# MartinMikkelsen/TensorTrainNumerics.jl

Hardware: AMD Instinct MI355X
Metric: TT cores/sec for QTT Laplacian apply+round, d=30 rank-64 (higher is better)
Workload: dtype f64

## Files before the change

tensortrainnumerics.jl_amd/csrc/ttn_eig_kernels.h:

```cpp
#pragma once
#include "ttn_dense_kernels.h"

#define EIG_N 128
template <int J>
__device__ __forceinline__ void fmac_bcast(double& a, double w, double s_) {
    asm volatile("v_fmac_f64_dpp %0, %1, %2 row_newbcast:%3 row_mask:0xf bank_mask:0xf" : "+v"(a) : "v"(w), "v"(s_), "n"(J));
}
#define EIG_BCAST16(M) M(0) M(1) M(2) M(3) M(4) M(5) M(6) M(7) M(8) M(9) M(10) M(11) M(12) M(13) M(14) M(15)
#define EIG_TAIL TTN_LDS_IMG

__device__ __forceinline__ void lds_barrier() { asm volatile("s_waitcnt lgkmcnt(0)\n\ts_barrier" ::: "memory"); }
__device__ __forceinline__ double wave64_sum_mfma(double v) {
    v = grp_sum(v);
    v += dpp_mov_f64<0x124>(v);
    v += dpp_mov_f64<0x128>(v);
    return v;
}
__device__ __forceinline__ double readlane_f64(double v, int idx) {
    union { double d; int i[2]; } u, r;
    u.d = v;
    r.i[0] = __builtin_amdgcn_readlane(u.i[0], idx);
    r.i[1] = __builtin_amdgcn_readlane(u.i[1], idx);
    return r.d;
}

template <int N>
__device__ __noinline__ void wg_tridiag(const double* Gg, int ldg, double* Vst, double* lds) {
    Gg = unip(Gg); Vst = unip(Vst); lds = unip(lds); ldg = uni32(ldg);
    constexpr bool TWO = (N == 128);
    constexpr int CW = (N * N / 16 > TTN_WG) ? 32 : 16;
    constexpr int NH = CW / 16;
    constexpr int NC = N / CW;
    static_assert(N * NC <= TTN_WG, "one thread per (row, column chunk)");
    lds_f64* L = (lds_f64*)lds;
    lds_f64 *vbuf0 = L, *vbuf1 = L + 128, *wL = L + 256, *xnext = L + 384, *part = L + 512;
    lds_f64 *dg = L + EIG_TAIL, *e = dg + 128, *beta = dg + 384;
    const int tid = threadIdx.x, lane = tid & 63, wave = tid >> 6;
    const int i = tid & (N - 1), c = tid / N;
    const bool actv = tid < N * NC;
    double a[CW];
#pragma unroll
    for (int j = 0; j < CW; ++j) a[j] = actv ? Gg[i + (long long)ldg * (CW * c + j)] : 0.0;
    lds_f64* xt = L + 1664;
    if (actv && i == 0) {
#pragma unroll
        for (int j = 0; j < CW; ++j) wL[CW * c + j] = a[j];
    }
    if (actv && i == 1) {
#pragma unroll
        for (int j = 0; j < CW; ++j) xnext[CW * c + j] = a[j];
    }
    __syncthreads();
    double rx0 = 0.0, rx1 = 0.0, ralpha = 0.0, rden = 0.0, rdg = 0.0;
    if (wave == 0) {
        rx0 = (lane > 0) ? wL[lane] : 0.0; rx1 = TWO ? wL[lane + 64] : 0.0;
        const double xk1 = wL[1];
        rdg = wL[0];
        xt[lane] = rx0; xt[lane + 64] = rx1;
        const double s2 = wave64_sum_mfma(fma(rx0, rx0, rx1 * rx1));
        ralpha = (s2 > 0.0) ? -copysign(s2 * fast_rsqrt2(s2), xk1) : 0.0;
        rden = s2 - ralpha * xk1;
    }
    for (int k = 0; k < N - 2; ++k) {
        lds_f64* vL = (k & 1) ? vbuf1 : vbuf0;
        lds_barrier();
        const bool live = actv && (CW * (c + 1) > k + 1) && ((TWO ? 64 * (wave & 1) : 0) + 63 > k);
        double v0 = 0.0, v1 = 0.0, w0 = 0.0, w1 = 0.0, bta = 0.0;
        if (wave == 0) {
            __builtin_amdgcn_s_setprio(TTN_TRIDIAG_PRIO);
            if (rden > 0.0) { bta = fast_rcp(rden); bta = fma(fma(-rden, bta, 1.0), bta, bta); }
            v0 = rx0 - ((lane == k + 1) ? ralpha : 0.0); v1 = rx1 - ((lane + 64 == k + 1) ? ralpha : 0.0);
            vL[lane] = v0; vL[lane + 64] = v1;
            typedef __attribute__((address_space(1))) double gdouble;
            gdouble* vg = (gdouble*)(unsigned long long)(Vst + k * 128);
            vg[lane] = v0; vg[lane + 64] = v1;
            if (lane == 0) { dg[k] = rdg; e[k] = ralpha; beta[k] = bta; }
        }
        if (live) {
            double xreg[NH];
#pragma unroll
            for (int h = 0; h < NH; ++h) xreg[h] = xt[CW * c + 16 * h + (lane & 15)];
            double pp = 0.0;
            asm volatile("s_nop 1");
#define EIG_MV(j) fmac_bcast<j>(pp, xreg[0], a[j]);
            EIG_BCAST16(EIG_MV)
#undef EIG_MV
            if constexpr (NH == 2) {
#define EIG_MV(j) fmac_bcast<j>(pp, xreg[1], a[16 + j]);
                EIG_BCAST16(EIG_MV)
#undef EIG_MV
            }
            part[c * 128 + i] = pp;
        } else if (actv) part[c * 128 + i] = 0.0;
        lds_barrier();
        lds_f64* xn_r = (k & 1) ? xnext + 1152 : xnext;
        lds_f64* xn_w = (k & 1) ? xnext : xnext + 1152;
        if (wave == 0) {
            double p0 = 0.0, p1 = 0.0;
#pragma unroll
            for (int cc = 0; cc < NC; ++cc) { p0 += part[cc * 128 + lane]; if (TWO) p1 += part[cc * 128 + lane + 64]; }
            p0 = bta * fma(-ralpha, xn_r[lane], p0); p1 = TWO ? bta * fma(-ralpha, xn_r[lane + 64], p1) : 0.0;
            const double Kc = 0.5 * bta * wave64_sum_mfma(fma(p0, v0, p1 * v1));
            w0 = fma(-Kc, v0, p0); w1 = fma(-Kc, v1, p1);
            wL[lane] = w0; if (TWO) wL[lane + 64] = w1;
        }
        lds_barrier();
        if (wave == 0 && k + 1 < N - 2) {
            const double wk1 = wL[k + 1], vk1 = vL[k + 1];
            const double c0 = fma(-v0, wk1, fma(-w0, vk1, xn_r[lane]));
            const double c1 = TWO ? fma(-v1, wk1, fma(-w1, vk1, xn_r[lane + 64])) : 0.0;
            const int kk = k + 1;
            rdg = (kk < 64) ? readlane_f64(c0, kk) : readlane_f64(c1, kk - 64);
            const double xk1 = (kk + 1 < 64) ? readlane_f64(c0, kk + 1) : readlane_f64(c1, kk + 1 - 64);
            rx0 = (lane > kk) ? c0 : 0.0; rx1 = (TWO && lane + 64 > kk) ? c1 : 0.0;
            xt[lane] = rx0; xt[lane + 64] = rx1;
            const double s2 = wave64_sum_mfma(fma(rx0, rx0, rx1 * rx1));
            ralpha = (s2 > 0.0) ? -copysign(s2 * fast_rsqrt2(s2), xk1) : 0.0;
            rden = s2 - ralpha * xk1;
        }
        if (wave == 0) __builtin_amdgcn_s_setprio(TTN_EIG_PRIO);
        if (live) {
            double vreg[NH], wreg[NH];
#pragma unroll
            for (int h = 0; h < NH; ++h) { vreg[h] = vL[CW * c + 16 * h + (lane & 15)]; wreg[h] = wL[CW * c + 16 * h + (lane & 15)]; }
            const double nvi = -vL[i], nwi = -wL[i];
            asm volatile("s_nop 1");
#define EIG_UP(j) fmac_bcast<j>(a[j], wreg[0], nvi); fmac_bcast<j>(a[j], vreg[0], nwi);
            EIG_BCAST16(EIG_UP)
#undef EIG_UP
            if constexpr (NH == 2) {
#define EIG_UP(j) fmac_bcast<j>(a[16 + j], wreg[1], nvi); fmac_bcast<j>(a[16 + j], vreg[1], nwi);
                EIG_BCAST16(EIG_UP)
#undef EIG_UP
            }
            if (i == k + 2) {
#pragma unroll
                for (int j = 0; j < CW; ++j) xn_w[CW * c + j] = a[j];
            }
        }
    }
    __syncthreads();
    if (actv && i == N - 2 && c == NC - 1) { dg[N - 2] = a[CW - 2]; e[N - 2] = a[CW - 1]; }
    if (actv && i == N - 1 && c == NC - 1) { dg[N - 1] = a[CW - 1]; }
    __syncthreads();
}

template <int N>
__device__ __forceinline__ int sturm_count(const double (&dreg)[N / 16], const double (&ereg)[N / 16], double x, bool& zero) {
    double pc = 1.0, pp = 0.0;
    const double nx = -x, one = 1.0;
    int cnt = 0;
    bool z = false;
    unsigned int prev = 0;
#pragma unroll
    for (int g = 0; g < N / 16; ++g) {
        unsigned int bits = 0;
#define EIG_ST(j) {                                                                                               \
            double dmx = nx;                                                                                      \
            fmac_bcast<j>(dmx, dreg[g], one);                                         \
            double pn = dmx * pc;                                                                                 \
            fmac_bcast<j>(pn, ereg[g], pp);                        \
            z |= (pn == 0.0);                                                                                     \
            bits = __builtin_amdgcn_alignbit(bits, (unsigned int)(__double_as_longlong(pn) >> 32), 31);           \
            pp = pc; pc = pn; }
        EIG_BCAST16(EIG_ST)
#undef EIG_ST
        const unsigned int seq = (prev << 16) | (bits & 0xffffu);
        cnt += __popc((seq ^ (seq >> 1)) & 0xffffu);
        prev = bits & 1u;
        const double ap = fabs(pc);
        if (ap < 0x1p-400 || ap > 0x1p400) {
            const double sc = (ap < 1.0) ? 0x1p500 : 0x1p-500;
            pc *= sc; pp *= sc;
        }
    }
    zero = z;
    return cnt;
}
__device__ __noinline__ int sturm_count_guarded(const lds_f64* de, double x, int n) {
    double pc = 1.0, pp = 0.0;
    int cnt = 0;
    for (int i = 0; i < n; ++i) {
        double pn = fma(de[2 * i] - x, pc, de[2 * i + 1] * pp);
        if (pn == 0.0) pn = copysign(DBL_MIN, -pc);
        cnt += (int)(((unsigned long long)(__double_as_longlong(pn) ^ __double_as_longlong(pc))) >> 63);
        pp = pc; pc = pn;
        const double ap = fabs(pc);
        if (ap < 0x1p-400 || ap > 0x1p400) { const double sc = (ap < 1.0) ? 0x1p500 : 0x1p-500; pc *= sc; pp *= sc; }
    }
    return cnt;
}

template <int N, int TL>
__device__ void wg_bisect(int nev, double* lds) {
    lds_f64* L = (lds_f64*)lds;
    lds_f64 *dg = L + EIG_TAIL, *e = dg + 128, *lam = dg + 256;
    lds_f64* e2 = L;
    const int tid = threadIdx.x;
    lds_f64* de = L + 256;
    for (int t = tid; t < N; t += TTN_WG) { e2[t] = (t < N - 1) ? e[t] * e[t] : 0.0; de[2 * t] = dg[t]; de[2 * t + 1] = (t > 0) ? -(e[t - 1] * e[t - 1]) : 0.0; }
    __syncthreads();
    if (tid < 64) {
        double glo_ = 1e300, ghi_ = -1e300, emax_ = 0.0;
        for (int t = tid; t < N; t += 64) {
            const double rad = ((t > 0) ? fabs(e[t - 1]) : 0.0) + ((t < N - 1) ? fabs(e[t]) : 0.0);
            glo_ = fmin(glo_, dg[t] - rad); ghi_ = fmax(ghi_, dg[t] + rad);
            emax_ = fmax(emax_, e2[t]);
        }
        glo_ = -wave_max(-glo_); ghi_ = wave_max(ghi_); emax_ = wave_max(emax_);
        if (tid == 0) { e2[128] = glo_; e2[129] = ghi_; e2[130] = emax_; }
    }
    __syncthreads();
    double glo = e2[128], ghi = e2[129];
    const double emax = e2[130];
    const double span = fmax(fabs(glo), fabs(ghi));
    glo -= 2.0 * DBL_EPSILON * span * N; ghi += 2.0 * DBL_EPSILON * span * N;
    const double pivmin = DBL_MIN * fmax(1.0, emax);
    double dreg[N / 16], ereg[N / 16];
#pragma unroll
    for (int g = 0; g < N / 16; ++g) { dreg[g] = de[2 * (16 * g + (tid & 15))]; ereg[g] = de[2 * (16 * g + (tid & 15)) + 1]; }
    asm volatile("s_nop 1");
    for (int g0 = 0; g0 < nev; g0 += TTN_WG / TL) {
        const int gi = g0 + tid / TL, sub = tid % TL;
        const bool act = gi < nev;
        const int jasc = N - 1 - (act ? gi : 0);
        double lo = glo, hi = ghi;
        for (int round = 0; round < 64; ++round) {
            const double wdt = hi - lo;
            const bool done = !(wdt > 2.0 * DBL_EPSILON * fmax(fabs(lo), fabs(hi)) + 2.0 * pivmin);
            if (__syncthreads_and(done || !act)) break;
            const double x = lo + wdt * ((double)(sub + 1) / (double)(TL + 1));
            const bool wave_act = g0 + (tid & ~63) / TL < nev;
            bool zero = false;
            int cnt = wave_act ? sturm_count<N>(dreg, ereg, x, zero) : 0;
            if (zero) cnt = sturm_count_guarded(de, x, N);
            int nf = (cnt <= jasc) ? 1 : 0;
#pragma unroll
            for (int m = 1; m < TL; m <<= 1) nf += __shfl_xor(nf, m);
            if (!done) {
                const double nlo = (nf > 0) ? lo + wdt * ((double)nf / (double)(TL + 1)) : lo;
                const double nhi = (nf < TL) ? lo + wdt * ((double)(nf + 1) / (double)(TL + 1)) : hi;
                lo = nlo; hi = nhi;
            }
        }
        if (act && sub == 0) lam[gi] = 0.5 * (lo + hi);
    }
    __syncthreads();
}

template <int N>
struct EigDm {
    static constexpr bool IN_LDS = 2 * N * 64 <= TTN_LDS_IMG;
    typedef __attribute__((address_space(1))) double gdouble;
    lds_f64* l;
    gdouble* g;
    __device__ __forceinline__ double ld(int idx) const { if constexpr (IN_LDS) return l[idx]; else return g[idx]; }
    __device__ __forceinline__ void st(int idx, double v) const { if constexpr (IN_LDS) l[idx] = v; else g[idx] = v; }
};
template <int N>
__device__ void wg_twisted(int r, double* lds, int* tw , lds_f64* zn , double* Dmg) {
    lds_f64* L = (lds_f64*)lds;
    lds_f64 *dg = L + EIG_TAIL, *e = dg + 128, *lam = dg + 256;
    lds_f64* Dp = L;
    EigDm<N> Dm;
    Dm.l = L + N * 64; Dm.g = (typename EigDm<N>::gdouble*)(unsigned long long)Dmg;
    const int tid = threadIdx.x, lane = tid & 63, wave = tid >> 6;
    double emax = 0.0;
    for (int t = 0; t < N - 1; ++t) emax = fmax(emax, e[t] * e[t]);
    const double pivmin = DBL_MIN * fmax(1.0, emax);
    __syncthreads();
    const bool act = lane < r;
    const double lm = lam[act ? lane : 0];
    if (wave == 0) {
        double q = 1.0;
        for (int i0 = 0; i0 < N; i0 += 8) {
            double dd[8], ee[8];
#pragma unroll
            for (int t = 0; t < 8; ++t) { dd[t] = dg[i0 + t]; ee[t] = (i0 + t > 0) ? e[i0 + t - 1] : 0.0; }
#pragma unroll
            for (int t = 0; t < 8; ++t) {
                q = fma(-(ee[t] * ee[t]), fast_rcp(q), dd[t] - lm);
                if (fabs(q) < pivmin) q = -pivmin;
                Dp[(i0 + t) * 64 + lane] = q;
            }
        }
    } else if (wave == 1) {
        double q = 1.0;
        for (int i0 = N - 8; i0 >= 0; i0 -= 8) {
            double dd[8], ee[8];
#pragma unroll
            for (int t = 0; t < 8; ++t) { dd[t] = dg[i0 + t]; ee[t] = (i0 + t < N - 1) ? e[i0 + t] : 0.0; }
#pragma unroll
            for (int t = 7; t >= 0; --t) {
                q = fma(-(ee[t] * ee[t]), fast_rcp(q), dd[t] - lm);
                if (fabs(q) < pivmin) q = -pivmin;
                Dm.st((i0 + t) * 64 + lane, q);
            }
        }
    }
    __syncthreads();
    if (wave < 2) {
        double gbest = 1e300;
        int kb = 0;
        for (int i0 = 0; i0 < N; i0 += 8) {
            double dm[8];
#pragma unroll
            for (int t = 0; t < 8; ++t) dm[t] = Dm.ld((i0 + t) * 64 + lane);
#pragma unroll
            for (int t = 0; t < 8; ++t) {
                const double g = fabs(Dp[(i0 + t) * 64 + lane] + dm[t] - (dg[i0 + t] - lm));
                if (g < gbest) { gbest = g; kb = i0 + t; }
            }
        }
        double z = 1.0, nrm = 0.0;
        if (wave == 0) {
            for (int i = kb - 1; i >= 0; --i) {
                z = -(e[i] * fast_rcp(Dp[i * 64 + lane])) * z;
                Dp[i * 64 + lane] = z;
                nrm = fma(z, z, nrm);
            }
            if (act) { tw[lane] = kb; zn[lane] = nrm; }
        } else {
            if constexpr (EigDm<N>::IN_LDS) {
                for (int i = kb; i < N - 1; ++i) {
                    z = -(e[i] * fast_rcp(Dm.ld((i + 1) * 64 + lane))) * z;
                    Dm.st((i + 1) * 64 + lane, z);
                    nrm = fma(z, z, nrm);
                }
            } else {
                for (int i0 = 0; i0 < N - 1; i0 += 8) {
                    double dm[8];
#pragma unroll
                    for (int t = 0; t < 8; ++t) dm[t] = (i0 + t + 1 < N) ? Dm.ld((i0 + t + 1) * 64 + lane) : 1.0;
#pragma unroll
                    for (int t = 0; t < 8; ++t) {
                        const int i = i0 + t;
                        if (i >= kb && i < N - 1) {
                            z = -(e[i] * fast_rcp(dm[t])) * z;
                            Dm.st((i + 1) * 64 + lane, z);
                            nrm = fma(z, z, nrm);
                        }
                    }
                }
            }
            if (act) zn[64 + lane] = nrm;
        }
    }
    __syncthreads();
    if (tid < 64 && tid < r) zn[tid] = 1.0 / sqrt(1.0 + zn[tid] + zn[64 + tid]);
    __syncthreads();
}

template <int N>
__device__ __noinline__ int wg_eig_n(const double* Gg, int ldg, double* Vst, int r, int nev, double* sig, double* lds, int* iwork ,
                                     double* dwork ) {
    Gg = unip(Gg); Vst = unip(Vst); sig = unip(sig); lds = unip(lds); iwork = unip(iwork); dwork = unip(dwork);
    r = uni32(r); nev = uni32(nev); ldg = uni32(ldg);
    constexpr int RPL = N / 16;
    lds_f64* L = (lds_f64*)lds;
    lds_f64 *lam = L + EIG_TAIL + 256, *beta = L + EIG_TAIL + 384;
    const int tid = threadIdx.x, lane = tid & 63, wave = tid >> 6;
    __builtin_amdgcn_s_setprio(TTN_EIG_PRIO);
    wg_tridiag<N>(Gg, ldg, Vst, lds);
    if (nev <= 32) wg_bisect<N, 8>(nev, lds);
    else wg_bisect<N, 4>(nev, lds);
    int bad = 0;
    for (int j = tid; j < nev; j += TTN_WG) { const double l = lam[j]; sig[j] = (l > 0.0) ? sqrt(l) : 0.0; bad |= (j < r) && !(l > 0.0); }
    if (__syncthreads_or(bad)) {
        __builtin_amdgcn_s_setprio(0); TTN_SETPRIO_BASE();
        return 1;
    }
    wg_twisted<N>(r, lds, iwork, (lds_f64*)dwork, const_cast<double*>(Gg));
    lds_f64* Dp = L;
    EigDm<N> Dm;
    Dm.l = L + N * 64; Dm.g = (typename EigDm<N>::gdouble*)(unsigned long long)Gg;
    const int rc = (lane & 3) | ((lane >> 4) << 2), col0 = 8 * (wave & 7) + 2 * ((lane >> 2) & 3);
    double z[2][RPL];
#pragma unroll
    for (int cc = 0; cc < 2; ++cc) {
        const int col = col0 + cc;
        const int kb = (col < r) ? iwork[col] : 0;
        const double zn = (col < r) ? ((lds_f64*)dwork)[col] : 0.0;
#pragma unroll
        for (int t = 0; t < RPL; ++t) {
            const int row = RPL * rc + t;
            const double v = (row < kb) ? Dp[row * 64 + col] : ((row == kb) ? 1.0 : Dm.ld(row * 64 + col));
            z[cc][t] = v * zn;
        }
    }
    constexpr int VROWS = TTN_LDS_IMG / 128;
    for (int khi = N - 2; khi > 0; khi -= VROWS) {
    const int klo = (khi > VROWS) ? khi - VROWS : 0;
    __syncthreads();
    wg_batched<8>((long long)(khi - klo) * 128, [&](long long e_) { return Vst[klo * 128 + e_]; }, [&](long long e_, double v) { L[e_] = v; });
    __syncthreads();
    if (wave < 8) {
        typedef double __attribute__((ext_vector_type(2))) d2;
        typedef __attribute__((address_space(3))) d2 lds_d2;
        for (int k = khi - 1; k >= klo; --k) {
            const lds_d2* vp = (const lds_d2*)(L + (k - klo) * 128 + RPL * rc);
            double vk[RPL];
#pragma unroll
            for (int t = 0; t < RPL / 2; ++t) { const d2 w2 = vp[t]; vk[2 * t] = w2.x; vk[2 * t + 1] = w2.y; }
            const double bk = beta[k];
            double s0 = 0.0, s1 = 0.0;
#pragma unroll
            for (int t = 0; t < RPL; ++t) { s0 = fma(vk[t], z[0][t], s0); s1 = fma(vk[t], z[1][t], s1); }
            const double t0 = grp_sum(s0) * bk, t1 = grp_sum(s1) * bk;
#pragma unroll
            for (int t = 0; t < RPL; ++t) { z[0][t] = fma(-t0, vk[t], z[0][t]); z[1][t] = fma(-t1, vk[t], z[1][t]); }
        }
    }
    }
    __syncthreads();
    if (wave < 8) {
#pragma unroll
        for (int cc = 0; cc < 2; ++cc) {
            const int col = col0 + cc;
            if (col < r) {
                const double sg = sig[col];
#pragma unroll
                for (int t = 0; t < RPL; ++t) L[col * 128 + RPL * rc + t] = z[cc][t] * sg;
            }
        }
    }
    __syncthreads();
    __builtin_amdgcn_s_setprio(0); TTN_SETPRIO_BASE();
    return 0;
}
__device__ int wg_eig128(const double* Gg, double* Vst, int r, int nev, double* sig, double* lds, int* iwork, double* dwork) {
    return wg_eig_n<128>(Gg, 128, Vst, r, nev, sig, lds, iwork, dwork);
}
__device__ int wg_eig64(const double* Gg, int ldg, double* Vst, int r, int nev, double* sig, double* lds, int* iwork, double* dwork) {
    return wg_eig_n<64>(Gg, ldg, Vst, r, nev, sig, lds, iwork, dwork);
}

__global__ void TTN_KERNEL_BOUNDS k_selftest_eig128(const double* G, double* Vst, int n, int r, int nev, double* sig, double* Xout, long long* clk) {
    extern __shared__ double lds[];
    int* iwork = reinterpret_cast<int*>(lds + GEMM_LDS_TOTAL + 32);
    double* dwork = lds + GEMM_LDS_TOTAL + 32 + 64;
    const long long t0 = (long long)__builtin_amdgcn_s_memtime();
    const int rc = (n == 64) ? wg_eig_n<64>(G, 64, Vst, r, nev, sig, lds, iwork, dwork) : wg_eig_n<128>(G, 128, Vst, r, nev, sig, lds, iwork, dwork);
    const long long t1 = (long long)__builtin_amdgcn_s_memtime();
    if (threadIdx.x == 0) { clk[0] = t1 - t0; clk[1] = rc; }
    if (rc == 0) for (int e = threadIdx.x; e < 128 * r; e += TTN_WG) Xout[e] = lds[e];
}
```

Baseline: 603,700.

## Apply Householder back-transform with blocked compact-WY T factors on MFMA

Replaces the one-reflector-at-a-time back-transformation of tridiagonal eigenvectors, which relied on scalar FMAs and group reductions, with a blocked compact-WY scheme. Idle waves build 16x16 T factors per reflector block during the twisted-factorization phase, and the update of the eigenvector matrix then runs as MFMA f64 16x16x4 products over staged reflector blocks in LDS. It also reuses emax computed in bisection instead of recomputing it serially. This adds global scratch traffic for T factors and more numerical reordering, and only the first 4 waves do the z update.

New measurement: 603,600. No clear change (-0.0%).

```diff
diff --git a/tensortrainnumerics.jl_amd/csrc/ttn_eig_kernels.h b/tensortrainnumerics.jl_amd/csrc/ttn_eig_kernels.h
--- a/tensortrainnumerics.jl_amd/csrc/ttn_eig_kernels.h
+++ b/tensortrainnumerics.jl_amd/csrc/ttn_eig_kernels.h
@@ -1,5 +1,6 @@
 #pragma once
 #include "ttn_dense_kernels.h"
+#include <type_traits>
 
 #define EIG_N 128
 template <int J>
@@ -8,6 +9,7 @@
 }
 #define EIG_BCAST16(M) M(0) M(1) M(2) M(3) M(4) M(5) M(6) M(7) M(8) M(9) M(10) M(11) M(12) M(13) M(14) M(15)
 #define EIG_TAIL TTN_LDS_IMG
+#define EIG_EMAX (EIG_TAIL + 511)
 
 __device__ __forceinline__ void lds_barrier() { asm volatile("s_waitcnt lgkmcnt(0)\n\ts_barrier" ::: "memory"); }
 __device__ __forceinline__ double wave64_sum_mfma(double v) {
@@ -208,7 +210,7 @@
             emax_ = fmax(emax_, e2[t]);
         }
         glo_ = -wave_max(-glo_); ghi_ = wave_max(ghi_); emax_ = wave_max(emax_);
-        if (tid == 0) { e2[128] = glo_; e2[129] = ghi_; e2[130] = emax_; }
+        if (tid == 0) { e2[128] = glo_; e2[129] = ghi_; e2[130] = emax_; L[EIG_EMAX] = emax_; }
     }
     __syncthreads();
     double glo = e2[128], ghi = e2[129];
@@ -257,16 +259,58 @@
     __device__ __forceinline__ double ld(int idx) const { if constexpr (IN_LDS) return l[idx]; else return g[idx]; }
     __device__ __forceinline__ void st(int idx, double v) const { if constexpr (IN_LDS) l[idx] = v; else g[idx] = v; }
 };
-template <int N>
-__device__ void wg_twisted(int r, double* lds, int* tw , lds_f64* zn , double* Dmg) {
+typedef __attribute__((address_space(1))) double eig_gdouble;
+template <int N>
+__device__ __forceinline__ int eig_tfac_off(int ldg, int b, int e) { return (e % N) + ldg * ((N == 128 ? 64 : 0) + b * (256 / N) + e / N); }
+__device__ __forceinline__ mfma_acc_t eig_prod16(mfma_acc_t xt, mfma_acc_t y, mfma_acc_t acc) {
+#pragma unroll
+    for (int s_ = 0; s_ < 4; ++s_) acc = __builtin_amdgcn_mfma_f64_16x16x4f64(xt[s_], y[s_], acc, 0, 0, 0);
+    return acc;
+}
+template <int N>
+__device__ __forceinline__ void wave_build_tfac(const double* Vst, const lds_f64* beta, eig_gdouble* Gt, int ldg, int b) {
+    const int lane = threadIdx.x & 63, li = lane & 15, lk = lane >> 4, k0 = 16 * b;
+    const bool kv = k0 + li < N - 2;
+    const eig_gdouble* vp = (const eig_gdouble*)(unsigned long long)(Vst + (kv ? k0 + li : 0) * 128 + lk);
+    const mfma_acc_t zero = (mfma_acc_t){0.0, 0.0, 0.0, 0.0};
+    mfma_acc_t sm = zero;
+    for (int q = k0 / 4; q < N / 4; q += 4) {
+        double a[4];
+#pragma unroll
+        for (int u = 0; u < 4; ++u) a[u] = kv ? vp[4 * (q + u)] : 0.0;
+#pragma unroll
+        for (int u = 0; u < 4; ++u) sm = __builtin_amdgcn_mfma_f64_16x16x4f64(a[u], a[u], sm, 0, 0, 0);
+    }
+    const double bj = kv ? beta[k0 + li] : 0.0;
+    mfma_acc_t m, mt, rr;
+#pragma unroll
+    for (int g = 0; g < 4; ++g) {
+        const int i = lk + 4 * g;
+        const double bi = (k0 + i < N - 2) ? beta[k0 + i] : 0.0;
+        m[g] = (i < li) ? -bi * sm[g] : 0.0;
+        mt[g] = (li < i) ? -bj * sm[g] : 0.0;
+        rr[g] = m[g] + ((i == li) ? 1.0 : 0.0);
+    }
+    const mfma_acc_t m2 = eig_prod16(mt, m, zero), m2t = eig_prod16(m, mt, zero);
+    const mfma_acc_t m4 = eig_prod16(m2t, m2, zero), m4t = eig_prod16(m2, m2t, zero);
+    const mfma_acc_t m8t = eig_prod16(m4, m4t, zero);
+    rr = eig_prod16(m2t, rr, rr);
+    rr = eig_prod16(m4t, rr, rr);
+    rr = eig_prod16(m8t, rr, rr);
+#pragma unroll
+    for (int g = 0; g < 4; ++g) Gt[eig_tfac_off<N>(ldg, b, 16 * li + lk + 4 * g)] = rr[g] * bj;
+}
+
+template <int N>
+__device__ void wg_twisted(int r, double* lds, int* tw , lds_f64* zn , double* Dmg, int ldg,
+                           const double* Vst) {
     lds_f64* L = (lds_f64*)lds;
     lds_f64 *dg = L + EIG_TAIL, *e = dg + 128, *lam = dg + 256;
     lds_f64* Dp = L;
     EigDm<N> Dm;
     Dm.l = L + N * 64; Dm.g = (typename EigDm<N>::gdouble*)(unsigned long long)Dmg;
     const int tid = threadIdx.x, lane = tid & 63, wave = tid >> 6;
-    double emax = 0.0;
-    for (int t = 0; t < N - 1; ++t) emax = fmax(emax, e[t] * e[t]);
+    const double emax = L[EIG_EMAX];
     const double pivmin = DBL_MIN * fmax(1.0, emax);
     __syncthreads();
     const bool act = lane < r;
@@ -297,6 +341,9 @@
                 Dm.st((i0 + t) * 64 + lane, q);
             }
         }
+    } else {
+        for (int b = wave - 2; b < (N - 2 + 15) / 16; b += TTN_WG / 64 - 2)
+            wave_build_tfac<N>(Vst, dg + 384, (eig_gdouble*)(unsigned long long)Dmg, ldg, b);
     }
     __syncthreads();
     if (wave < 2) {
@@ -370,58 +417,82 @@
         __builtin_amdgcn_s_setprio(0); TTN_SETPRIO_BASE();
         return 1;
     }
-    wg_twisted<N>(r, lds, iwork, (lds_f64*)dwork, const_cast<double*>(Gg));
+    wg_twisted<N>(r, lds, iwork, (lds_f64*)dwork, const_cast<double*>(Gg), ldg, Vst);
     lds_f64* Dp = L;
     EigDm<N> Dm;
     Dm.l = L + N * 64; Dm.g = (typename EigDm<N>::gdouble*)(unsigned long long)Gg;
-    const int rc = (lane & 3) | ((lane >> 4) << 2), col0 = 8 * (wave & 7) + 2 * ((lane >> 2) & 3);
-    double z[2][RPL];
-#pragma unroll
-    for (int cc = 0; cc < 2; ++cc) {
-        const int col = col0 + cc;
+    const eig_gdouble* Tg = (const eig_gdouble*)(unsigned long long)Gg;
+    constexpr int RT = N / 16, NB = (N - 2 + 15) / 16;
+    constexpr int LDV = 130;
+    constexpr int CB0 = GEMM_LDS_DOUBLES / (16 * LDV), CB = CB0 < NB ? CB0 : NB;
+    static_assert(CB >= RT / 4 && CB * 16 * LDV <= GEMM_LDS_DOUBLES, "staged reflector blocks fit the image + tail");
+    const int li = lane & 15, lk = lane >> 4, col = 16 * wave + li;
+    const bool zwave = wave < 4 && 16 * wave < r;
+    mfma_acc_t z[RT];
+    if (zwave) {
         const int kb = (col < r) ? iwork[col] : 0;
         const double zn = (col < r) ? ((lds_f64*)dwork)[col] : 0.0;
 #pragma unroll
-        for (int t = 0; t < RPL; ++t) {
-            const int row = RPL * rc + t;
-            const double v = (row < kb) ? Dp[row * 64 + col] : ((row == kb) ? 1.0 : Dm.ld(row * 64 + col));
-            z[cc][t] = v * zn;
-        }
-    }
-    constexpr int VROWS = TTN_LDS_IMG / 128;
-    for (int khi = N - 2; khi > 0; khi -= VROWS) {
-    const int klo = (khi > VROWS) ? khi - VROWS : 0;
-    __syncthreads();
-    wg_batched<8>((long long)(khi - klo) * 128, [&](long long e_) { return Vst[klo * 128 + e_]; }, [&](long long e_, double v) { L[e_] = v; });
-    __syncthreads();
-    if (wave < 8) {
-        typedef double __attribute__((ext_vector_type(2))) d2;
-        typedef __attribute__((address_space(3))) d2 lds_d2;
-        for (int k = khi - 1; k >= klo; --k) {
-            const lds_d2* vp = (const lds_d2*)(L + (k - klo) * 128 + RPL * rc);
-            double vk[RPL];
-#pragma unroll
-            for (int t = 0; t < RPL / 2; ++t) { const d2 w2 = vp[t]; vk[2 * t] = w2.x; vk[2 * t + 1] = w2.y; }
-            const double bk = beta[k];
-            double s0 = 0.0, s1 = 0.0;
-#pragma unroll
-            for (int t = 0; t < RPL; ++t) { s0 = fma(vk[t], z[0][t], s0); s1 = fma(vk[t], z[1][t], s1); }
-            const double t0 = grp_sum(s0) * bk, t1 = grp_sum(s1) * bk;
-#pragma unroll
-            for (int t = 0; t < RPL; ++t) { z[0][t] = fma(-t0, vk[t], z[0][t]); z[1][t] = fma(-t1, vk[t], z[1][t]); }
-        }
-    }
-    }
-    __syncthreads();
-    if (wave < 8) {
-#pragma unroll
-        for (int cc = 0; cc < 2; ++cc) {
-            const int col = col0 + cc;
-            if (col < r) {
-                const double sg = sig[col];
-#pragma unroll
-                for (int t = 0; t < RPL; ++t) L[col * 128 + RPL * rc + t] = z[cc][t] * sg;
-            }
+        for (int t = 0; t < RT; ++t) {
+#pragma unroll
+            for (int g = 0; g < 4; ++g) {
+                const int row = 16 * t + lk + 4 * g;
+                const double v = (row < kb) ? Dp[row * 64 + col] : ((row == kb) ? 1.0 : Dm.ld(row * 64 + col));
+                z[t][g] = (col < r) ? v * zn : 0.0;
+            }
+        }
+    }
+    auto block_step = [&](auto t0_, int b, const lds_f64* Vb) {
+        constexpr int T0 = decltype(t0_)::value;
+        double ta[4];
+#pragma unroll
+        for (int s_ = 0; s_ < 4; ++s_) ta[s_] = Tg[eig_tfac_off<N>(ldg, b, 16 * (lk + 4 * s_) + li)];
+        const mfma_acc_t zero = (mfma_acc_t){0.0, 0.0, 0.0, 0.0};
+        mfma_acc_t y = zero;
+#pragma unroll
+        for (int t = T0; t < RT; ++t) {
+#pragma unroll
+            for (int g = 0; g < 4; ++g) y = __builtin_amdgcn_mfma_f64_16x16x4f64(Vb[li * LDV + 16 * t + 4 * g + lk], z[t][g], y, 0, 0, 0);
+        }
+        mfma_acc_t w = zero;
+#pragma unroll
+        for (int s_ = 0; s_ < 4; ++s_) w = __builtin_amdgcn_mfma_f64_16x16x4f64(ta[s_], y[s_], w, 0, 0, 0);
+#pragma unroll
+        for (int s_ = 0; s_ < 4; ++s_) {
+            const double nw = -w[s_];
+#pragma unroll
+            for (int t = T0; t < RT; ++t) z[t] = __builtin_amdgcn_mfma_f64_16x16x4f64(Vb[(4 * s_ + lk) * LDV + 16 * t + li], nw, z[t], 0, 0, 0);
+        }
+    };
+#pragma nounroll
+    for (int bhi = NB; bhi > 0; bhi -= CB) {
+        const int blo = (bhi > CB) ? bhi - CB : 0, klo = 16 * blo;
+        __syncthreads();
+        wg_batched<8>((long long)(bhi - blo) * 16 * N,
+                      [&](long long e_) { const int k = klo + (int)e_ / N; return (k < N - 2) ? Vst[k * 128 + (int)e_ % N] : 0.0; },
+                      [&](long long e_, double v) { L[((int)e_ / N) * LDV + (int)e_ % N] = v; });
+        __syncthreads();
+        if (zwave) {
+#pragma nounroll
+            for (int b = bhi - 1; b >= blo; --b) {
+                const lds_f64* Vb = L + (16 * b - klo) * LDV;
+                if (b >= RT / 2) block_step(std::integral_constant<int, RT / 2>{}, b, Vb);
+                else block_step(std::integral_constant<int, 0>{}, b, Vb);
+            }
+        }
+    }
+    __syncthreads();
+    if (zwave) {
+        double sg[4];
+#pragma unroll
+        for (int g = 0; g < 4; ++g) { const int c = 16 * wave + lk + 4 * g; sg[g] = (c < r) ? sig[c] : 0.0; }
+#pragma unroll
+        for (int t = 0; t < RT; ++t) {
+            mfma_acc_t zt = (mfma_acc_t){0.0, 0.0, 0.0, 0.0};
+#pragma unroll
+            for (int s_ = 0; s_ < 4; ++s_) zt = __builtin_amdgcn_mfma_f64_16x16x4f64(z[t][s_], (lk + 4 * s_ == li) ? 1.0 : 0.0, zt, 0, 0, 0);
+#pragma unroll
+            for (int g = 0; g < 4; ++g) { const int c = 16 * wave + lk + 4 * g; if (c < r) L[c * 128 + 16 * t + li] = zt[g] * sg[g]; }
         }
     }
     __syncthreads();
```
